# aikiriao/AAD

Measured on AMD Instinct MI355X. Metric: Msamples/s encode+decode, 48 kHz stereo 4-bit, higher is better.
Workload: dtype int32

## Files before the change

### aad_amd/capi.py

```python
import ctypes as C
import os

import numpy as np


class AADApiResult:
    OK = 0
    INVALID_ARGUMENT = 1
    INVALID_FORMAT = 2
    INSUFFICIENT_BUFFER = 3
    INSUFFICIENT_DATA = 4
    PARAMETER_NOT_SET = 5
    NG = 6
    _names = {0: "OK", 1: "INVALID_ARGUMENT", 2: "INVALID_FORMAT", 3: "INSUFFICIENT_BUFFER",
              4: "INSUFFICIENT_DATA", 5: "PARAMETER_NOT_SET", 6: "NG"}

    @classmethod
    def name(cls, v):
        return cls._names.get(int(v), str(v))


class AADHeaderInfo(C.Structure):
    _fields_ = [("format_version", C.c_uint32), ("codec_version", C.c_uint32),
                ("num_channels", C.c_uint16), ("num_samples", C.c_uint32),
                ("sampling_rate", C.c_uint32), ("bits_per_sample", C.c_uint16),
                ("block_size", C.c_uint16), ("num_samples_per_block", C.c_uint32),
                ("ch_process_method", C.c_int)]


class AADEncodeParameter(C.Structure):
    _fields_ = [("num_channels", C.c_uint16), ("sampling_rate", C.c_uint32),
                ("bits_per_sample", C.c_uint16), ("max_block_size", C.c_uint16),
                ("ch_process_method", C.c_int), ("num_encode_trials", C.c_uint8)]


class AADHipStreamDesc(C.Structure):
    _fields_ = [("pcm_offset", C.c_uint64), ("data_offset", C.c_uint64),
                ("data_size", C.c_uint64), ("num_samples", C.c_uint32), ("reserved", C.c_uint32)]


class AADHipSegmentation(C.Structure):
    _fields_ = [("segment_blocks", C.c_uint32), ("warmup_blocks", C.c_uint32)]


class AADHipPlanarLayout(C.Structure):
    _fields_ = [("sample_type", C.c_int32), ("reserved", C.c_uint32), ("channel_stride", C.c_uint64)]


class AADHipPlanarOutput(C.Structure):
    _fields_ = [("sample_type", C.c_int32), ("reserved", C.c_uint32), ("stream_stride", C.c_uint64), ("channel_stride", C.c_uint64)]


class AADHipRowStats(C.Structure):
    _fields_ = [("sum_sq", C.c_uint64), ("sum_abs", C.c_uint64), ("max_abs", C.c_uint64), ("count", C.c_uint64)]


class AADHipLaneState(C.Structure):
    _fields_ = [("weight", C.c_int32 * 4), ("history", C.c_int32 * 4),
                ("stepsize_index", C.c_int32), ("quantize_error", C.c_int32)]


STREAM_DESC_DTYPE = np.dtype([("pcm_offset", "<u8"), ("data_offset", "<u8"), ("data_size", "<u8"),
                              ("num_samples", "<u4"), ("reserved", "<u4")])
ERROR_STATS_DTYPE = np.dtype([("rms_error", "<f8"), ("mean_abs_error", "<f8"), ("max_abs_error", "<f8")])
WINDOW_DTYPE = np.dtype([("stream", "<i8"), ("first_frame", "<i8")])
SAMPLE_INT16, SAMPLE_FLOAT32 = 0, 1
RECONSTRUCT_DECODED, RECONSTRUCT_RESIDUAL = 0, 1
OPTION_LANE_MAPPING, OPTION_TRIAL_LANES, OPTION_STAGING_THREADS, OPTION_TILE_KBYTES, OPTION_COMPARE_ORDER = 0, 1, 2, 3, 4
LANE_MAPPINGS = {"auto": 0, "dense": 1, "quad": 2, "quad-fused": 3, "dense-tiled": 4}
TRIAL_LANES = {"dual": 0, "single": 1}
OPTION_SIMD_ROLE = 5
SIMD_ROLE_OFF = -1
LANE_STATE_DTYPE = np.dtype([("weight", "<i4", (4,)), ("history", "<i4", (4,)),
                             ("stepsize_index", "<i4"), ("quantize_error", "<i4")])

_PKG_DIR = os.path.dirname(os.path.abspath(__file__))
LIBRARY_PATH = os.environ.get("AAD_HIP_LIBRARY", os.path.join(_PKG_DIR, "libaad_hip.so"))

LEGACY_SYMBOLS = [
    "AADEncoder_CalculateBlockSize", "AADEncoder_EncodeHeader", "AADEncoder_CalculateWorkSize",
    "AADEncoder_Create", "AADEncoder_Destroy", "AADEncoder_SetEncodeParameter", "AADEncoder_EncodeWhole",
    "AADDecoder_DecodeHeader", "AADDecoder_CalculateWorkSize", "AADDecoder_Create", "AADDecoder_Destroy",
    "AADDecoder_SetHeader", "AADDecoder_DecodeBlock", "AADDecoder_DecodeWhole",
]
HIP_SYMBOLS = [
    "AADHip_GetDeviceCount", "AADHip_ContextCreate", "AADHip_ContextDestroy", "AADHip_ContextSynchronize",
    "AADHip_ContextLastError", "AADHip_ContextSignalNextRun", "AADHip_SignalNextRunSupported", "AADHip_ContextSetOption", "AADHip_CalculateEncodedSize", "AADHip_EncodePlanCreate",
    "AADHip_EncodePlanDestroy", "AADHip_EncodePlanRun", "AADHip_DecodePlanCreate", "AADHip_DecodePlanDestroy",
    "AADHip_DecodePlanRun", "AADHip_EncodeBatch", "AADHip_DecodeBatch",
    "AADHip_ReconstructPlanCreate", "AADHip_ReconstructPlanDestroy", "AADHip_ReconstructPlanRun",
    "AADHip_ReconstructBatch", "AADHip_SegmentedEncodePlanCreate", "AADHip_SegmentedEncodeBatch",
    "AADHip_SegmentedReconstructPlanCreate", "AADHip_SegmentedReconstructBatch",
    "AADHip_WindowDecodePlanCreate", "AADHip_WindowDecodePlanDestroy", "AADHip_WindowDecodePlanRun",
    "AADHip_WindowDecodePlanRunStats", "AADHip_MixedWindowDecodePlanCreate", "AADHip_ChannelMixWindowDecodePlanCreate",
    "AADHip_PlanarEncodePlanCreate", "AADHip_PlanarEncodePlanRun",
    "AADHip_PlanarReconstructPlanCreate", "AADHip_PlanarReconstructPlanRun", "AADHip_PlanarReconstructPlanRunStats",
    "AADHip_WindowReconstructPlanCreate", "AADHip_WindowReconstructPlanDestroy", "AADHip_WindowReconstructPlanRun",
]
WAV_SYMBOLS = ["AADWav_ParseHeader", "AADWav_WriteHeader", "AADWav_ConvertToPcm16"]
SYNTH_SYMBOLS = ["AADSynth_Generate"]


class AADWavInfo(C.Structure):
    _fields_ = [("format_tag", C.c_uint16), ("num_channels", C.c_uint16), ("sampling_rate", C.c_uint32),
                ("bits_per_sample", C.c_uint16), ("num_samples", C.c_uint32), ("data_offset", C.c_uint64),
                ("data_size", C.c_uint64)]


def _declare_legacy(lib):
    u8p, i32pp = C.POINTER(C.c_uint8), C.POINTER(C.POINTER(C.c_int32))
    lib.AADEncoder_CalculateBlockSize.argtypes = [C.c_uint16, C.c_uint16, C.c_uint32,
                                                  C.POINTER(C.c_uint16), C.POINTER(C.c_uint32)]
    lib.AADEncoder_CalculateBlockSize.restype = C.c_int
    lib.AADEncoder_EncodeHeader.argtypes = [C.POINTER(AADHeaderInfo), u8p, C.c_uint32]
    lib.AADEncoder_EncodeHeader.restype = C.c_int
    lib.AADEncoder_CalculateWorkSize.argtypes = [C.c_uint16]
    lib.AADEncoder_CalculateWorkSize.restype = C.c_int32
    lib.AADEncoder_Create.argtypes = [C.c_uint16, C.c_void_p, C.c_int32]
    lib.AADEncoder_Create.restype = C.c_void_p
    lib.AADEncoder_Destroy.argtypes = [C.c_void_p]
    lib.AADEncoder_Destroy.restype = None
    lib.AADEncoder_SetEncodeParameter.argtypes = [C.c_void_p, C.POINTER(AADEncodeParameter)]
    lib.AADEncoder_SetEncodeParameter.restype = C.c_int
    lib.AADEncoder_EncodeWhole.argtypes = [C.c_void_p, i32pp, C.c_uint32, u8p, C.c_uint32, C.POINTER(C.c_uint32)]
    lib.AADEncoder_EncodeWhole.restype = C.c_int
    lib.AADDecoder_DecodeHeader.argtypes = [u8p, C.c_uint32, C.POINTER(AADHeaderInfo)]
    lib.AADDecoder_DecodeHeader.restype = C.c_int
    lib.AADDecoder_CalculateWorkSize.argtypes = []
    lib.AADDecoder_CalculateWorkSize.restype = C.c_int32
    lib.AADDecoder_Create.argtypes = [C.c_void_p, C.c_int32]
    lib.AADDecoder_Create.restype = C.c_void_p
    lib.AADDecoder_Destroy.argtypes = [C.c_void_p]
    lib.AADDecoder_Destroy.restype = None
    lib.AADDecoder_SetHeader.argtypes = [C.c_void_p, C.POINTER(AADHeaderInfo)]
    lib.AADDecoder_SetHeader.restype = C.c_int
    lib.AADDecoder_DecodeBlock.argtypes = [C.c_void_p, u8p, C.c_uint32, i32pp, C.c_uint32, C.c_uint32,
                                           C.POINTER(C.c_uint32)]
    lib.AADDecoder_DecodeBlock.restype = C.c_int
    lib.AADDecoder_DecodeWhole.argtypes = [C.c_void_p, u8p, C.c_uint32, i32pp, C.c_uint32, C.c_uint32]
    lib.AADDecoder_DecodeWhole.restype = C.c_int


def _declare_hip(lib):
    vp = C.c_void_p
    lib.AADHip_GetDeviceCount.argtypes = []
    lib.AADHip_GetDeviceCount.restype = C.c_int32
    lib.AADHip_ContextCreate.argtypes = [C.c_int32, vp, C.POINTER(vp)]
    lib.AADHip_ContextCreate.restype = C.c_int
    lib.AADHip_ContextDestroy.argtypes = [vp]
    lib.AADHip_ContextDestroy.restype = None
    lib.AADHip_ContextSynchronize.argtypes = [vp]
    lib.AADHip_ContextSynchronize.restype = C.c_int
    lib.AADHip_ContextLastError.argtypes = [vp]
    lib.AADHip_ContextLastError.restype = C.c_char_p
    lib.AADHip_ContextSignalNextRun.argtypes = [vp, vp, vp]
    lib.AADHip_ContextSignalNextRun.restype = C.c_int
    lib.AADHip_SignalNextRunSupported.argtypes = []
    lib.AADHip_SignalNextRunSupported.restype = C.c_int32
    lib.AADHip_ContextSetOption.argtypes = [vp, C.c_int32, C.c_int32]
    lib.AADHip_ContextSetOption.restype = C.c_int
    lib.AADHip_CalculateEncodedSize.argtypes = [C.POINTER(AADEncodeParameter), C.c_uint32]
    lib.AADHip_CalculateEncodedSize.restype = C.c_uint64
    lib.AADHip_EncodePlanCreate.argtypes = [vp, C.POINTER(AADEncodeParameter), C.c_uint32, vp, C.POINTER(vp)]
    lib.AADHip_EncodePlanCreate.restype = C.c_int
    lib.AADHip_SegmentedEncodePlanCreate.argtypes = [vp, C.POINTER(AADEncodeParameter), C.POINTER(AADHipSegmentation), C.c_uint32, vp,
                                                     C.POINTER(vp)]
    lib.AADHip_SegmentedEncodePlanCreate.restype = C.c_int
    lib.AADHip_PlanarEncodePlanCreate.argtypes = [vp, C.POINTER(AADEncodeParameter), C.POINTER(AADHipPlanarLayout),
                                                  C.POINTER(AADHipSegmentation), C.c_uint32, vp, C.POINTER(vp)]
    lib.AADHip_PlanarEncodePlanCreate.restype = C.c_int
    lib.AADHip_PlanarEncodePlanRun.argtypes = [vp, vp, vp, vp]
    lib.AADHip_PlanarEncodePlanRun.restype = C.c_int
    lib.AADHip_PlanarReconstructPlanCreate.argtypes = [vp, C.POINTER(AADEncodeParameter), C.POINTER(AADHipPlanarLayout),
                                                       C.POINTER(AADHipPlanarOutput), C.POINTER(AADHipSegmentation), C.c_uint32, vp,
                                                       C.POINTER(vp)]
    lib.AADHip_PlanarReconstructPlanCreate.restype = C.c_int
    lib.AADHip_PlanarReconstructPlanRun.argtypes = [vp, vp, vp, vp, vp]
    lib.AADHip_PlanarReconstructPlanRun.restype = C.c_int
    lib.AADHip_PlanarReconstructPlanRunStats.argtypes = [vp, vp, vp, vp, vp, vp]
    lib.AADHip_PlanarReconstructPlanRunStats.restype = C.c_int
    lib.AADHip_WindowReconstructPlanCreate.argtypes = [vp, C.POINTER(AADEncodeParameter), C.POINTER(AADHipPlanarLayout),
                                                       C.POINTER(AADHipSegmentation), C.c_uint32, vp, C.POINTER(vp)]
    lib.AADHip_WindowReconstructPlanCreate.restype = C.c_int
    lib.AADHip_WindowReconstructPlanDestroy.argtypes = [vp]
    lib.AADHip_WindowReconstructPlanDestroy.restype = None
    lib.AADHip_WindowReconstructPlanRun.argtypes = [vp, vp, C.c_uint64, vp, C.c_uint32, C.c_uint64, vp, C.POINTER(AADHipPlanarOutput),
                                                    vp, vp]
    lib.AADHip_WindowReconstructPlanRun.restype = C.c_int
    lib.AADHip_EncodePlanDestroy.argtypes = [vp]
    lib.AADHip_EncodePlanDestroy.restype = None
    lib.AADHip_EncodePlanRun.argtypes = [vp, vp, vp, vp]
    lib.AADHip_EncodePlanRun.restype = C.c_int
    lib.AADHip_DecodePlanCreate.argtypes = [vp, C.POINTER(AADHeaderInfo), C.c_int32, C.c_uint32, vp, C.POINTER(vp)]
    lib.AADHip_DecodePlanCreate.restype = C.c_int
    lib.AADHip_DecodePlanDestroy.argtypes = [vp]
    lib.AADHip_DecodePlanDestroy.restype = None
    lib.AADHip_DecodePlanRun.argtypes = [vp, vp, vp]
    lib.AADHip_DecodePlanRun.restype = C.c_int
    lib.AADHip_WindowDecodePlanCreate.argtypes = [vp, C.POINTER(AADHeaderInfo), C.c_int32, C.c_uint32, vp, C.POINTER(vp)]
    lib.AADHip_WindowDecodePlanCreate.restype = C.c_int
    lib.AADHip_MixedWindowDecodePlanCreate.argtypes = [vp, C.c_uint32, C.c_int32, C.c_uint32, vp, vp, C.POINTER(vp)]
    lib.AADHip_MixedWindowDecodePlanCreate.restype = C.c_int
    lib.AADHip_ChannelMixWindowDecodePlanCreate.argtypes = [vp, C.c_uint32, C.c_int32, C.c_uint32, vp, vp, C.POINTER(vp)]
    lib.AADHip_ChannelMixWindowDecodePlanCreate.restype = C.c_int
    lib.AADHip_WindowDecodePlanDestroy.argtypes = [vp]
    lib.AADHip_WindowDecodePlanDestroy.restype = None
    lib.AADHip_WindowDecodePlanRun.argtypes = [vp, vp, C.c_uint64, vp, C.c_uint32, C.c_int32, vp]
    lib.AADHip_WindowDecodePlanRun.restype = C.c_int
    lib.AADHip_WindowDecodePlanRunStats.argtypes = [vp, vp, C.c_uint64, vp, C.c_uint32, C.c_int32, vp, vp]
    lib.AADHip_WindowDecodePlanRunStats.restype = C.c_int
    lib.AADHip_EncodeBatch.argtypes = [vp, C.POINTER(AADEncodeParameter), C.c_uint32, vp, vp, vp, vp, vp, vp]
    lib.AADHip_EncodeBatch.restype = C.c_int
    lib.AADHip_DecodeBatch.argtypes = [vp, C.c_uint32, vp, vp, vp, vp, vp]
    lib.AADHip_DecodeBatch.restype = C.c_int
    lib.AADHip_ReconstructPlanCreate.argtypes = [vp, C.POINTER(AADEncodeParameter), C.c_uint32, vp, C.POINTER(vp)]
    lib.AADHip_ReconstructPlanCreate.restype = C.c_int
    lib.AADHip_ReconstructPlanDestroy.argtypes = [vp]
    lib.AADHip_ReconstructPlanDestroy.restype = None
    lib.AADHip_ReconstructPlanRun.argtypes = [vp, vp, vp, vp, C.c_int32, vp]
    lib.AADHip_ReconstructPlanRun.restype = C.c_int
    lib.AADHip_ReconstructBatch.argtypes = [vp, C.POINTER(AADEncodeParameter), C.c_uint32, vp, vp, C.c_int32, vp, vp]
    lib.AADHip_ReconstructBatch.restype = C.c_int
    lib.AADHip_SegmentedEncodeBatch.argtypes = [vp, C.POINTER(AADEncodeParameter), C.POINTER(AADHipSegmentation), C.c_uint32, vp, vp,
                                                vp, vp, vp]
    lib.AADHip_SegmentedEncodeBatch.restype = C.c_int
    lib.AADHip_SegmentedReconstructPlanCreate.argtypes = [vp, C.POINTER(AADEncodeParameter), C.POINTER(AADHipSegmentation), C.c_uint32,
                                                          vp, C.POINTER(vp)]
    lib.AADHip_SegmentedReconstructPlanCreate.restype = C.c_int
    lib.AADHip_SegmentedReconstructBatch.argtypes = [vp, C.POINTER(AADEncodeParameter), C.POINTER(AADHipSegmentation), C.c_uint32, vp,
                                                     vp, C.c_int32, vp, vp]
    lib.AADHip_SegmentedReconstructBatch.restype = C.c_int
    lib.AADWav_ParseHeader.argtypes = [vp, C.c_uint64, C.POINTER(AADWavInfo)]
    lib.AADWav_ParseHeader.restype = C.c_int
    lib.AADWav_WriteHeader.argtypes = [vp, C.c_uint32, C.c_uint16, C.c_uint32, C.c_uint32]
    lib.AADWav_WriteHeader.restype = C.c_int
    lib.AADWav_ConvertToPcm16.argtypes = [vp, C.c_uint16, C.c_uint64, vp]
    lib.AADWav_ConvertToPcm16.restype = C.c_int


def load_library(path=None, hip=True):
    path = path or LIBRARY_PATH
    if not os.path.exists(path):
        raise FileNotFoundError(
            "%s is missing - the HIP extension has not been built (run __graft_entry__.build())" % path)
    if hip:
        try:
            import torch
        except ImportError:
            pass
    lib = C.CDLL(path)
    _declare_legacy(lib)
# ... 101 lines not shown
```

### aad_amd/csrc/aad_hip_engine.hip

```cpp
#include <hip/hip_runtime.h>

#include <cstdio>
#include <cstdlib>
#include <cstring>
#include <algorithm>
#include <condition_variable>
#include <functional>
#include <mutex>
#include <new>
#include <thread>
#include <vector>

#include "../../include/aad_hip.h"
#include "aad_compare.hip.h"
#include "aad_launch.h"
#include "aad_decode.hip.h"
#include "aad_decode_window.hip.h"
#include "aad_decode_window_mixed.hip.h"
#include "aad_decode_window_channel_mix.hip.h"
#include "aad_encode.hip.h"
#include "aad_encode_launch.hip.h"
#include "aad_format.h"
#include "aad_hip_internal.h"
#include "aad_tiles.h"
#include "aad_window_reconstruct.hip.h"

namespace aad {
thread_local LaunchSignal tl_launch_signal = {nullptr, nullptr};
}

static_assert(sizeof(AADHipStreamDesc) == sizeof(aad::StreamDesc), "stream table layout");
static_assert(sizeof(AADHipLaneState) == sizeof(aad::LaneStateRecord), "lane state layout");
static_assert(sizeof(AADHipErrorStats) == sizeof(aad::ErrorStatsRecord), "error stats layout");

struct Staging {
  void *host = nullptr, *dev = nullptr;
  size_t cap = 0;
};

struct StagingPool {
  std::vector<std::thread> threads;
  std::mutex lock;
  std::condition_variable work, done;
  std::function<void(unsigned)> job;
  unsigned generation = 0, pending = 0;
  bool stop = false;
};

struct AADHipContext {
  int device;
  hipStream_t stream;
  bool owns_stream;
  char last_error[256];
  Staging in[2], out[2];
  hipEvent_t chunk_done[2];
  hipEvent_t piece_done[3];
  hipStream_t up_stream, down_stream;
  hipEvent_t uploaded[2], computed[2];
  bool have_events, have_pipeline;
  void *d_rc_in, *d_rc_out;
  size_t rc_in_capacity, rc_out_capacity;
  void *d_scratch;
  size_t scratch_capacity;
  int32_t *d_residual;
  uint64_t residual_capacity;
  uint8_t *d_trial;
  uint64_t trial_capacity;
  uint8_t *d_window_images;
  uint64_t window_images_capacity;
  aad::LaunchSignal signal_next;
  bool signal_refused;
  aad::Device device_info;
  aad::Knobs knobs;
  int32_t compare_sequential;
  int64_t tile_bytes;
  void *d_state;
// ... 2188 lines not shown
  if (num_streams == 0) return AAD_APIRESULT_OK;
  for (uint32_t i = 0; i < num_streams; i++)
    if (pcm[i] == nullptr || (out_pcm != nullptr && out_pcm[i] == nullptr)) return AAD_APIRESULT_INVALID_ARGUMENT;
  AADHeaderInfo h;
  std::vector<uint64_t> sizes, footprint(num_streams);
  const AADApiResult checked = host_encode_check(parameter, num_streams, num_samples, nullptr, &h, &sizes);
  if (checked != AAD_APIRESULT_OK) return checked;
  for (uint32_t i = 0; i < num_streams; i++) footprint[i] = reconstruct_footprint(num_samples[i], h.num_channels, sizes[i]);
  if (segmentation != nullptr) {
    std::vector<AADHipStreamDesc> streams(num_streams);
    for (uint32_t i = 0; i < num_streams; i++) streams[i] = AADHipStreamDesc{0, 0, 0, num_samples[i], 0};
    if (aad::segment_chain_count(streams.data(), num_streams, h.num_samples_per_block, segmentation->segment_blocks) > UINT32_MAX) {
      snprintf(ctx->last_error, sizeof(ctx->last_error), "segmented reconstruction: more than %u chains", (unsigned)UINT32_MAX);
      return AAD_APIRESULT_INVALID_ARGUMENT;
    }
  }
  const uint64_t chunk = staging_chunk(ctx);
  uint64_t budget;
  if (!wave_budget(ctx, &budget)) return AAD_APIRESULT_NG;
  AADApiResult rc = AAD_APIRESULT_OK;
  for (uint32_t first = 0; first < num_streams && rc == AAD_APIRESULT_OK;) {
    uint32_t n = 0;
    uint64_t sum = 0;
    while (first + n < num_streams && (n == 0 || sum + footprint[first + n] <= budget)) sum += footprint[first + n++];
    rc = reconstruct_wave(ctx, parameter, segmentation, n, pcm + first, num_samples + first, output_kind, out_pcm ? out_pcm + first : nullptr,
                          stats ? stats + first : nullptr, chunk);
    first += n;
  }
  return rc;
}

}

AADApiResult AADHip_ReconstructBatch(struct AADHipContext *ctx, const struct AADEncodeParameter *parameter,
                                     uint32_t num_streams, const int16_t *const *pcm, const uint32_t *num_samples,
                                     int32_t output_kind, int16_t *const *out_pcm, struct AADHipErrorStats *stats)
{
  if (ctx == nullptr || parameter == nullptr || (num_streams != 0 && (pcm == nullptr || num_samples == nullptr)))
    return AAD_APIRESULT_INVALID_ARGUMENT;
  return reconstruct_batch(ctx, parameter, nullptr, num_streams, pcm, num_samples, output_kind, out_pcm, stats);
}

AADApiResult AADHip_SegmentedReconstructBatch(struct AADHipContext *ctx, const struct AADEncodeParameter *parameter,
                                              const struct AADHipSegmentation *segmentation, uint32_t num_streams,
                                              const int16_t *const *pcm, const uint32_t *num_samples, int32_t output_kind,
                                              int16_t *const *out_pcm, struct AADHipErrorStats *stats)
{
  if (ctx == nullptr || parameter == nullptr || segmentation == nullptr || segmentation->segment_blocks == 0 ||
      (num_streams != 0 && (pcm == nullptr || num_samples == nullptr)))
    return AAD_APIRESULT_INVALID_ARGUMENT;
  return reconstruct_batch(ctx, parameter, segmentation, num_streams, pcm, num_samples, output_kind, out_pcm, stats);
}

#if AAD_PHASE_TIMING
uint32_t AADHipDebug_ReadPhaseTimes(uint64_t *out, uint32_t capacity)
{
  uint32_t n = 0, zero = 0;
  uint64_t host[512];
  (void)hipDeviceSynchronize();
  (void)hipMemcpyFromSymbol(&n, HIP_SYMBOL(aad::g_phase_count), sizeof(n));
  (void)hipMemcpyFromSymbol(host, HIP_SYMBOL(aad::g_phase_times), sizeof(host));
  (void)hipMemcpyToSymbol(HIP_SYMBOL(aad::g_phase_count), &zero, sizeof(zero));
  if (n > capacity) n = capacity;
  memcpy(out, host, sizeof(uint64_t) * n);
  return n;
}
#endif

}
```

### aad_amd/csrc/aad_launch_policy.h

```cpp
#ifndef AAD_LAUNCH_POLICY_H
#define AAD_LAUNCH_POLICY_H

#include <stdint.h>

#include "../../include/aad_hip.h"
#include "aad_lds_layout.h"

namespace aad {

struct Device {
  uint32_t cus, lds_per_cu;
};

struct Knobs {
  int32_t lane_mapping = AAD_HIP_LANE_MAPPING_AUTO;
  int32_t trial_lanes = AAD_HIP_TRIAL_LANES_DUAL;
  int32_t encode_ring = 1;
  int32_t encode_lds_pad = -1;
  int32_t decode_lds_pad = -1;
  uint64_t decode_nt_min = 0;
  int32_t simd_role = AAD_HIP_SIMD_ROLE_OFF;
};

struct EncodeBatch {
// ... 368 lines not shown
  uint32_t channels, bits, mid_side, min_samples_per_block, streams;
};
constexpr uint32_t kMaxChannelMixVariants = 9;
struct ChannelMixVariants {
  uint32_t count;
  ChannelMixVariant v[kMaxChannelMixVariants];
};

inline ChannelMixVariants channel_mix_variants(const ChannelStreamFormat *formats, uint64_t n)
{
  ChannelMixVariant slot[kMaxChannelMixVariants] = {};
  for (uint64_t i = 0; i < n; i++) {
    const ChannelStreamFormat &f = formats[i];
    if (f.bits < 2 || f.bits > 4 || f.source >= kSourceNone) continue;
    const bool mono = f.source == kSourceMono, ms = f.source == kSourceMidSide;
    ChannelMixVariant &s = slot[mono ? 6u + (4u - f.bits) : (4u - f.bits) * 2u + (ms ? 1u : 0u)];
    if (s.streams == 0 || f.samples_per_block < s.min_samples_per_block) s.min_samples_per_block = f.samples_per_block;
    s.channels = mono ? 1u : 2u;
    s.bits = f.bits;
    s.mid_side = ms ? 1u : 0u;
    s.streams++;
  }
  ChannelMixVariants out = {};
  for (const ChannelMixVariant &s : slot)
    if (s.streams != 0) out.v[out.count++] = s;
  return out;
}

struct ChannelMixWindowLaunch {
  bool ok;
  uint32_t count;
  ChannelMixVariant variant[kMaxChannelMixVariants];
  WindowLaunch launch[kMaxChannelMixVariants];
};

inline ChannelMixWindowLaunch plan_channel_mix_window_decode(const Device &d, const Knobs &k, const ChannelMixVariants &variants,
                                                             uint64_t windows, uint32_t frames, uint32_t out_channels)
{
  ChannelMixWindowLaunch m = {};
  ChannelMixVariants vs = variants;
  if (vs.count == 0) vs.v[vs.count++] = ChannelMixVariant{1, 4, 0, frames, 0};
  if (vs.count > kMaxChannelMixVariants || out_channels < 1 || out_channels > 2) return m;
  for (uint32_t i = 0; i < vs.count; i++) {
    m.variant[i] = vs.v[i];
    m.launch[i] = plan_window_decode_into(d, k, WindowBatch{windows, frames, vs.v[i].channels, vs.v[i].bits, vs.v[i].min_samples_per_block},
                                          out_channels);
    if (!m.launch[i].ok) return m;
  }
  m.count = vs.count;
  m.ok = true;
  return m;
}

}

#endif
```

### aad_amd/engine.py

```python
import ctypes as C

import numpy as np

from .capi import (AADApiResult, AADHeaderInfo, AADHipPlanarLayout, AADHipPlanarOutput, AADHipSegmentation, ApiError, ERROR_STATS_DTYPE, LANE_MAPPINGS, LANE_STATE_DTYPE,
                   OPTION_COMPARE_ORDER, OPTION_LANE_MAPPING, OPTION_SIMD_ROLE, OPTION_STAGING_THREADS, OPTION_TILE_KBYTES, OPTION_TRIAL_LANES, RECONSTRUCT_DECODED, RECONSTRUCT_RESIDUAL,
                   SAMPLE_FLOAT32, SAMPLE_INT16, SIMD_ROLE_OFF, STREAM_DESC_DTYPE, TRIAL_LANES, WINDOW_DTYPE, load_library, make_parameter)


def _check(where, rc):
    if rc != AADApiResult.OK:
        raise ApiError(where, rc)


def _round_up(v, a):
    return (v + a - 1) // a * a


class Engine:

    def __init__(self, device=0, stream="torch", lib=None):
        import torch
        if not torch.cuda.is_available():
            raise RuntimeError("aad_amd.Engine needs a HIP device (torch.cuda.is_available() is False)")
        self.torch = torch
        self.lib = lib or load_library()
        self.device = int(device)
        torch.cuda.set_device(self.device)
        if stream == "torch":
            cur = torch.cuda.current_stream(self.device)
            self.stream = cur if cur.cuda_stream != 0 else torch.cuda.Stream(self.device)
        elif stream is None:
            self.stream = torch.cuda.Stream(self.device)
        else:
            self.stream = stream
        self._ctx = C.c_void_p()
        _check("AADHip_ContextCreate",
               self.lib.AADHip_ContextCreate(self.device, self.stream.cuda_stream, C.byref(self._ctx)))

    def _enter(self):
        cur = self.torch.cuda.current_stream(self.device)
        if cur.cuda_stream != self.stream.cuda_stream:
            self.stream.wait_stream(cur)
        return cur

    def _exit(self, cur):
        if cur.cuda_stream != self.stream.cuda_stream:
            cur.wait_stream(self.stream)

    def close(self):
        if self._ctx:
            self.lib.AADHip_ContextDestroy(self._ctx)
            self._ctx = C.c_void_p()

    def __del__(self):
        try:
            self.close()
        except Exception:
            pass

# ... 799 lines not shown
        if self.handle:
            self.runtime().hipEventDestroy(self.handle)
            self.handle = C.c_void_p()

    def __del__(self):
        try:
            self.close()
        except Exception:
            pass


PIPELINE_SIMD_ROLES = True


class SimdRoleAllocator:
    SLOTS = ((0, 1), (2, 3))

    def __init__(self):
        self.taken = [False] * len(self.SLOTS)
        self.holders = [None] * len(self.SLOTS)

    def in_force(self):
        return all(self.taken)

    def acquire(self, apply=None):
        for i, t in enumerate(self.taken):
            if not t:
                self.taken[i] = True
                self.holders[i] = apply
                self._apply_all()
                return i
        return None

    def release(self, slot):
        if slot is not None and self.taken[slot]:
            apply = self.holders[slot]
            self.taken[slot], self.holders[slot] = False, None
            if apply is not None:
                apply(None, None)
            self._apply_all()

    def roles(self, slot):
        return self.SLOTS[slot] if slot is not None and self.taken[slot] and self.in_force() else (None, None)

    def _apply_all(self):
        for i, apply in enumerate(self.holders):
            if self.taken[i] and apply is not None:
                apply(*self.roles(i))


_simd_roles = {}


class EncodeDecodePipeline:

    def __init__(self, enc_engine, dec_engine, param, streams, samples, ring=8, simd_roles=PIPELINE_SIMD_ROLES):
        assert ring >= 2 and ring % 2 == 0
        assert enc_engine.stream.cuda_stream != dec_engine.stream.cuda_stream, "the two contexts need streams of their own"
        torch = enc_engine.torch
        self.torch, self.ring, self.k = torch, ring, 0
        self.enc_engine, self.dec_engine = enc_engine, dec_engine
        self._take_simd_roles(_simd_roles.setdefault(enc_engine.device, SimdRoleAllocator()) if simd_roles else None)
        self.enc = enc_engine.uniform_encode_plan(param, streams, samples)
        self.images = [torch.zeros((streams, self.enc.stride), dtype=torch.uint8, device="cuda:%d" % enc_engine.device)
                       for _ in range(ring)]
        zero = torch.zeros((streams, samples, param.num_channels), dtype=torch.int16, device=self.images[0].device)
        self.enc.run(zero, self.images[0])
        torch.cuda.synchronize()
        self.header = parse_header(bytes(self.images[0][0, :31].cpu().numpy()))
        self.dec = dec_engine.uniform_decode_plan(self.header, streams, self.enc.stride, self.enc.image_size)
        self.encoded = [HipEvent() for _ in range(ring)]
        self.decoded = [torch.cuda.Event() for _ in range(ring)]

    def step(self, pcm, out, timing=None):
        k, ring = self.k, self.ring
        self.k += 1
        b = k % ring
        s_enc, s_dec = self.enc_engine.stream, self.dec_engine.stream
        if k >= ring and k % (ring // 2) == 0:
            s_enc.wait_event(self.decoded[(k - ring // 2 - 1) % ring])
        encoded = self.encoded[b] if timing is None else timing[1]
        self.enc_engine.signal_next(encoded, start=None if timing is None else timing[0])
        self.enc.run(pcm, self.images[b], None, ordered=False)
        encoded.wait_on(s_dec)
        if timing is not None:
            self.dec_engine.signal_next(timing[3], start=timing[2])
        self.dec.run(self.images[b], out, ordered=False)
        self.decoded[b].record(s_dec)
        return self.images[b]

    def close(self):
        self.torch.cuda.synchronize()
        self.enc.close()
        self.dec.close()
        for e in self.encoded:
            e.close()
        self._release_simd_roles()

    def _take_simd_roles(self, allocator):
        self._roles = allocator
        self._role_slot = allocator.acquire(self._set_simd_roles) if allocator is not None else None

    def _set_simd_roles(self, enc_simd, dec_simd):
        self.enc_engine.set_simd_role(enc_simd)
        self.dec_engine.set_simd_role(dec_simd)

    def _release_simd_roles(self):
        if getattr(self, "_role_slot", None) is not None:
            self._roles.release(self._role_slot)
            self._role_slot = None


def parse_header(data):
    if len(data) < 31 or data[:4] != b"AAD\x00":
        raise ApiError("parse_header", AADApiResult.INVALID_FORMAT)
    be = lambda o, n: int.from_bytes(data[o:o + n], "big")
    return AADHeaderInfo(format_version=be(4, 4), codec_version=be(8, 4), num_channels=be(12, 2),
                         num_samples=be(14, 4), sampling_rate=be(18, 4), bits_per_sample=be(22, 2),
                         block_size=be(24, 2), num_samples_per_block=be(26, 4), ch_process_method=data[30])


__all__ = ["Engine", "EncodePlan", "PlanarEncodePlan", "PlanarReconstructPlan", "DecodePlan", "WindowDecodePlan", "EncodeDecodePipeline", "SimdRoleAllocator", "parse_header", "make_parameter", "LANE_STATE_DTYPE", "rmse", "snr_db", "level_dbfs", "select_least_bits"]
```

### include/aad_hip.h

```cpp
#ifndef AAD_HIP_H_INCLUDED
#define AAD_HIP_H_INCLUDED

#include <stdint.h>
#include "aad.h"
#include "aad_encoder.h"

#define AAD_HIP_MAX_NUM_CHANNELS 8

struct AADHipContext;
struct AADHipEncodePlan;
struct AADHipDecodePlan;

struct AADHipStreamDesc {
  uint64_t pcm_offset;
  uint64_t data_offset;
  uint64_t data_size;
  uint32_t num_samples;
  uint32_t reserved;
};

struct AADHipLaneState {
  int32_t weight[4];
  int32_t history[4];
  int32_t stepsize_index;
// ... 22 lines not shown
  AAD_HIP_OPTION_COMPARE_ORDER = 4,
  AAD_HIP_OPTION_SIMD_ROLE = 5
};
enum AADHipSimdRole {
  AAD_HIP_SIMD_ROLE_OFF = -1,
  AAD_HIP_SIMD_ROLE_0 = 0, AAD_HIP_SIMD_ROLE_1 = 1, AAD_HIP_SIMD_ROLE_2 = 2, AAD_HIP_SIMD_ROLE_3 = 3
};
enum AADHipLaneMapping {
  AAD_HIP_LANE_MAPPING_AUTO = 0,
  AAD_HIP_LANE_MAPPING_DENSE = 1,
  AAD_HIP_LANE_MAPPING_QUAD = 2,
  AAD_HIP_LANE_MAPPING_QUAD_FUSED = 3,
  AAD_HIP_LANE_MAPPING_DENSE_TILED = 4
};
enum AADHipTrialLanes {
  AAD_HIP_TRIAL_LANES_DUAL = 0,
  AAD_HIP_TRIAL_LANES_SINGLE = 1
};
AADApiResult AADHip_ContextSetOption(struct AADHipContext *context, int32_t option, int32_t value);

uint64_t AADHip_CalculateEncodedSize(const struct AADEncodeParameter *parameter, uint32_t num_samples);


AADApiResult AADHip_EncodePlanCreate(
    struct AADHipContext *context, const struct AADEncodeParameter *parameter,
    uint32_t num_streams, const struct AADHipStreamDesc *streams,
    struct AADHipEncodePlan **plan);
void AADHip_EncodePlanDestroy(struct AADHipEncodePlan *plan);

AADApiResult AADHip_EncodePlanRun(
    struct AADHipEncodePlan *plan, const int16_t *device_pcm, uint8_t *device_data,
    struct AADHipLaneState *device_state);


struct AADHipSegmentation {
  uint32_t segment_blocks;
  uint32_t warmup_blocks;
};
AADApiResult AADHip_SegmentedEncodePlanCreate(
    struct AADHipContext *context, const struct AADEncodeParameter *parameter,
    const struct AADHipSegmentation *segmentation,
    uint32_t num_streams, const struct AADHipStreamDesc *streams,
    struct AADHipEncodePlan **plan);


AADApiResult AADHip_DecodePlanCreate(
    struct AADHipContext *context, const struct AADHeaderInfo *format, int32_t has_file_header,
    uint32_t num_streams, const struct AADHipStreamDesc *streams,
    struct AADHipDecodePlan **plan);
void AADHip_DecodePlanDestroy(struct AADHipDecodePlan *plan);

AADApiResult AADHip_DecodePlanRun(
    struct AADHipDecodePlan *plan, const uint8_t *device_data, int16_t *device_pcm);


struct AADHipWindow {
  uint64_t stream;
  uint64_t first_frame;
};
enum AADHipSampleType {
  AAD_HIP_SAMPLE_INT16 = 0,
  AAD_HIP_SAMPLE_FLOAT32 = 1
};
struct AADHipWindowDecodePlan;
AADApiResult AADHip_WindowDecodePlanCreate(
    struct AADHipContext *context, const struct AADHeaderInfo *format, int32_t has_file_header,
    uint32_t num_streams, const struct AADHipStreamDesc *streams,
    struct AADHipWindowDecodePlan **plan);
void AADHip_WindowDecodePlanDestroy(struct AADHipWindowDecodePlan *plan);
AADApiResult AADHip_WindowDecodePlanRun(
    struct AADHipWindowDecodePlan *plan, const uint8_t *device_data,
    uint64_t num_windows, const struct AADHipWindow *device_windows,
    uint32_t frames_per_window, int32_t sample_type, void *device_out);

AADApiResult AADHip_MixedWindowDecodePlanCreate(
    struct AADHipContext *context, uint32_t num_channels, int32_t has_file_header,
    uint32_t num_streams, const struct AADHipStreamDesc *streams,
    const struct AADHeaderInfo *formats,
    struct AADHipWindowDecodePlan **plan);

AADApiResult AADHip_ChannelMixWindowDecodePlanCreate(
    struct AADHipContext *context, uint32_t out_channels , int32_t has_file_header,
    uint32_t num_streams, const struct AADHipStreamDesc *streams,
    const struct AADHeaderInfo *formats,
    struct AADHipWindowDecodePlan **plan);

struct AADHipRowStats;
AADApiResult AADHip_WindowDecodePlanRunStats(
    struct AADHipWindowDecodePlan *plan, const uint8_t *device_data,
    uint64_t num_windows, const struct AADHipWindow *device_windows,
    uint32_t frames_per_window, int32_t sample_type,
    void *device_out,
    struct AADHipRowStats *device_stats);


struct AADHipPlanarLayout {
  int32_t sample_type;
  uint32_t reserved;
  uint64_t channel_stride;
};
AADApiResult AADHip_PlanarEncodePlanCreate(
    struct AADHipContext *context, const struct AADEncodeParameter *parameter,
    const struct AADHipPlanarLayout *layout,
    const struct AADHipSegmentation *segmentation,
    uint32_t num_streams, const struct AADHipStreamDesc *streams,
    struct AADHipEncodePlan **plan);
// ... 114 lines not shown
```

Measured before the change: 120,000.

## Move encode/decode step pipeline into native code with alternate-stream ordering

Adds a native StepPipeline that schedules encode and decode across two HIP streams with ring-slot events. Per-step Python stream and event bookkeeping is replaced by one C call. A planner picks an 'alternate' order, which runs encode and decode back-to-back on one stream and alternates streams per step, when both kernels would use no more workgroups than there are CUs. Otherwise it keeps the prior overlap order. This cuts host overhead and cross-stream waits when kernels are too small to fill the GPU, at the cost of extra plans and more complex ordering logic.

```diff
diff --git a/aad_amd/capi.py b/aad_amd/capi.py
--- a/aad_amd/capi.py
+++ b/aad_amd/capi.py
@@ -71,6 +71,7 @@
 TRIAL_LANES = {"dual": 0, "single": 1}
 OPTION_SIMD_ROLE = 5
 SIMD_ROLE_OFF = -1
+STEP_ORDERS = {"auto": -1, "overlap": 0, "alternate": 1}
 LANE_STATE_DTYPE = np.dtype([("weight", "<i4", (4,)), ("history", "<i4", (4,)),
                              ("stepsize_index", "<i4"), ("quantize_error", "<i4")])
 
@@ -96,6 +97,8 @@
     "AADHip_PlanarEncodePlanCreate", "AADHip_PlanarEncodePlanRun",
     "AADHip_PlanarReconstructPlanCreate", "AADHip_PlanarReconstructPlanRun", "AADHip_PlanarReconstructPlanRunStats",
     "AADHip_WindowReconstructPlanCreate", "AADHip_WindowReconstructPlanDestroy", "AADHip_WindowReconstructPlanRun",
+    "AADHip_StepPipelineCreate", "AADHip_StepPipelineRun", "AADHip_StepPipelineDestroy", "AADHip_StepPipelineOrder",
+    "AADHip_StepPipelineImageStride", "AADHip_StepPipelineEncodePlan", "AADHip_StepPipelineDecodePlan",
 ]
 WAV_SYMBOLS = ["AADWav_ParseHeader", "AADWav_WriteHeader", "AADWav_ConvertToPcm16"]
 SYNTH_SYMBOLS = ["AADSynth_Generate"]
@@ -197,6 +200,21 @@
     lib.AADHip_DecodePlanDestroy.restype = None
     lib.AADHip_DecodePlanRun.argtypes = [vp, vp, vp]
     lib.AADHip_DecodePlanRun.restype = C.c_int
+    lib.AADHip_StepPipelineCreate.argtypes = [vp, vp, C.POINTER(AADEncodeParameter), C.c_uint32, C.c_uint32, C.c_uint32, C.POINTER(vp),
+                                              C.c_int32, C.POINTER(vp)]
+    lib.AADHip_StepPipelineCreate.restype = C.c_int
+    lib.AADHip_StepPipelineRun.argtypes = [vp, vp, vp, C.POINTER(vp), C.POINTER(C.c_uint32)]
+    lib.AADHip_StepPipelineRun.restype = C.c_int
+    lib.AADHip_StepPipelineDestroy.argtypes = [vp]
+    lib.AADHip_StepPipelineDestroy.restype = None
+    lib.AADHip_StepPipelineOrder.argtypes = [vp]
+    lib.AADHip_StepPipelineOrder.restype = C.c_int32
+    lib.AADHip_StepPipelineImageStride.argtypes = [vp]
+    lib.AADHip_StepPipelineImageStride.restype = C.c_uint64
+    lib.AADHip_StepPipelineEncodePlan.argtypes = [vp, C.c_uint32]
+    lib.AADHip_StepPipelineEncodePlan.restype = vp
+    lib.AADHip_StepPipelineDecodePlan.argtypes = [vp, C.c_uint32]
+    lib.AADHip_StepPipelineDecodePlan.restype = vp
     lib.AADHip_WindowDecodePlanCreate.argtypes = [vp, C.POINTER(AADHeaderInfo), C.c_int32, C.c_uint32, vp, C.POINTER(vp)]
     lib.AADHip_WindowDecodePlanCreate.restype = C.c_int
     lib.AADHip_MixedWindowDecodePlanCreate.argtypes = [vp, C.c_uint32, C.c_int32, C.c_uint32, vp, vp, C.POINTER(vp)]
diff --git a/aad_amd/csrc/aad_hip_engine.hip b/aad_amd/csrc/aad_hip_engine.hip
--- a/aad_amd/csrc/aad_hip_engine.hip
+++ b/aad_amd/csrc/aad_hip_engine.hip
@@ -22,6 +22,7 @@
 #include "aad_encode_launch.hip.h"
 #include "aad_format.h"
 #include "aad_hip_internal.h"
+#include "aad_step_schedule.h"
 #include "aad_tiles.h"
 #include "aad_window_reconstruct.hip.h"
 
@@ -2316,6 +2317,193 @@
   return reconstruct_batch(ctx, parameter, segmentation, num_streams, pcm, num_samples, output_kind, out_pcm, stats);
 }
 
+
+struct AADHipStepPipeline {
+  AADHipContext *ctx[2];
+  AADHipEncodePlan *enc[2];
+  AADHipDecodePlan *dec[2];
+  aad::StepOrder order;
+  uint32_t ring;
+  uint64_t k, stride, out_elements;
+  std::vector<uint8_t *> images;
+  std::vector<hipEvent_t> own[2];
+  std::vector<hipEvent_t> done[2];
+  const int16_t *last_out;
+};
+
+namespace {
+
+void step_pipeline_free(AADHipStepPipeline *p)
+{
+  for (int q = 0; q < 2; q++) {
+    AADHip_EncodePlanDestroy(p->enc[q]);
+    AADHip_DecodePlanDestroy(p->dec[q]);
+  }
+  for (auto &events : p->own)
+    for (hipEvent_t e : events)
+      if (e != nullptr) (void)hipEventDestroy(e);
+  delete p;
+}
+
+AADApiResult step_pipeline_launch(AADHipStepPipeline *p, aad::StepKernel kernel, uint32_t queue, uint32_t slot, hipEvent_t start,
+                                  hipEvent_t stop, const int16_t *device_pcm, int16_t *device_out)
+{
+  const AADApiResult rc = AADHip_ContextSignalNextRun(p->ctx[queue], start, stop);
+  if (rc != AAD_APIRESULT_OK) return rc;
+  p->done[(int)kernel][slot] = stop;
+  return kernel == aad::StepKernel::Encode ? AADHip_EncodePlanRun(p->enc[queue], device_pcm, p->images[slot], nullptr)
+                                           : AADHip_DecodePlanRun(p->dec[queue], p->images[slot], device_out);
+}
+
+}
+
+AADApiResult AADHip_StepPipelineCreate(struct AADHipContext *ctx0, struct AADHipContext *ctx1, const struct AADEncodeParameter *parameter,
+                                       uint32_t num_streams, uint32_t num_samples, uint32_t ring, uint8_t *const *device_images,
+                                       int32_t order, struct AADHipStepPipeline **pipeline)
+{
+  if (pipeline == nullptr) return AAD_APIRESULT_INVALID_ARGUMENT;
+  *pipeline = nullptr;
+  if (ctx0 == nullptr || ctx1 == nullptr || ctx0 == ctx1 || parameter == nullptr || device_images == nullptr || num_streams == 0 ||
+      !aad::step_ring_ok(ring) || order < AAD_HIP_STEP_ORDER_AUTO || order > AAD_HIP_STEP_ORDER_ALTERNATE)
+    return AAD_APIRESULT_INVALID_ARGUMENT;
+  if (ctx0->device != ctx1->device || ctx0->stream == ctx1->stream) return AAD_APIRESULT_INVALID_ARGUMENT;
+  for (uint32_t i = 0; i < ring; i++)
+    if (device_images[i] == nullptr) return AAD_APIRESULT_INVALID_ARGUMENT;
+  if (ctx0->signal_refused || ctx1->signal_refused) {
+    snprintf(ctx0->last_error, sizeof(ctx0->last_error),
+             "AADHip_StepPipelineCreate: refused, ROC_SYSTEM_SCOPE_SIGNAL=0 (the pipeline orders its two streams with the kernels' own "
+             "completion signals, AADHip_ContextSignalNextRun)");
+    return AAD_APIRESULT_NG;
+  }
+  AADHeaderInfo header;
+  if (AADFormat_ParameterToHeader(parameter, num_samples, AAD_HIP_MAX_NUM_CHANNELS, &header) != AAD_APIRESULT_OK ||
+      !AADFormat_HeaderFieldsValid(&header, AAD_HIP_MAX_NUM_CHANNELS))
+    return AAD_APIRESULT_INVALID_FORMAT;
+  const uint64_t image_size = AADHip_CalculateEncodedSize(parameter, num_samples);
+  if (image_size == 0) return AAD_APIRESULT_INVALID_FORMAT;
+  const uint64_t stride = (image_size + 63u) / 64u * 64u;
+  std::vector<AADHipStreamDesc> table(num_streams);
+  for (uint32_t i = 0; i < num_streams; i++)
+    table[i] = AADHipStreamDesc{(uint64_t)i * num_samples * parameter->num_channels, (uint64_t)i * stride, stride, num_samples, 0};
+
+  AADHipStepPipeline *p = new (std::nothrow) AADHipStepPipeline();
+  if (p == nullptr) return AAD_APIRESULT_NG;
+  p->ctx[0] = ctx0;
+  p->ctx[1] = ctx1;
+  p->ring = ring;
+  p->stride = stride;
+  p->out_elements = (uint64_t)num_streams * num_samples * parameter->num_channels;
+  p->images.assign(device_images, device_images + ring);
+  AADApiResult rc = AADHip_EncodePlanCreate(ctx0, parameter, num_streams, table.data(), &p->enc[0]);
+  for (auto &d : table) d.data_size = image_size;
+  if (rc == AAD_APIRESULT_OK) rc = AADHip_DecodePlanCreate(ctx1, &header, 1, num_streams, table.data(), &p->dec[1]);
+  if (rc == AAD_APIRESULT_OK) {
+    const aad::EncodeArgs &e = p->enc[0]->run.args;
+    const aad::DecodeArgs &d = p->dec[1]->args;
+    p->order = (aad::StepOrder)aad::plan_step_order(
+        ctx0->device_info, ctx0->knobs, aad::EncodeBatch{e.bits, e.channels, e.num_streams, e.trials, e.block_size, e.ring_ok != 0},
+        aad::DecodeBatch{d.total_blocks, d.num_streams, d.channels, d.bits, d.samples_per_block, d.block_size, d.code_phase_uniform,
+                         d.pcm_aligned16 != 0, true, d.stream_stores != 0},
+        order);
+    if (p->order == aad::StepOrder::Alternate) {
+      rc = AADHip_DecodePlanCreate(ctx0, &header, 1, num_streams, table.data(), &p->dec[0]);
+      for (auto &t : table) t.data_size = stride;
+      if (rc == AAD_APIRESULT_OK) rc = AADHip_EncodePlanCreate(ctx1, parameter, num_streams, table.data(), &p->enc[1]);
+    }
+  }
+  if (rc == AAD_APIRESULT_OK) {
+    DeviceGuard guard(ctx0);
+    bool ok = guard.ok;
+    for (int kernel = 0; kernel < 2 && ok; kernel++) {
+      p->own[kernel].assign(ring, nullptr);
+      p->done[kernel].assign(ring, nullptr);
+      for (uint32_t i = 0; i < ring && ok; i++)
+        ok = hip_ok(ctx0, hipEventCreateWithFlags(&p->own[kernel][i], hipEventDisableTiming), "hipEventCreateWithFlags");
+    }
+    if (!ok) rc = AAD_APIRESULT_NG;
+  }
+  if (rc != AAD_APIRESULT_OK) {
+    step_pipeline_free(p);
+    return rc;
+  }
+  *pipeline = p;
+  return AAD_APIRESULT_OK;
+}
+
+AADApiResult AADHip_StepPipelineRun(struct AADHipStepPipeline *p, const int16_t *device_pcm, int16_t *device_out,
+                                    void *const *timing_events, uint32_t *slot)
+{
+  if (p == nullptr || device_pcm == nullptr || device_out == nullptr) return AAD_APIRESULT_INVALID_ARGUMENT;
+  hipEvent_t timing[4] = {nullptr, nullptr, nullptr, nullptr};
+  if (timing_events != nullptr)
+    for (int i = 0; i < 4; i++) {
+      if (timing_events[i] == nullptr) return AAD_APIRESULT_INVALID_ARGUMENT;
+      timing[i] = static_cast<hipEvent_t>(timing_events[i]);
+    }
+  const uint64_t k = p->k;
+  const bool overlaps = p->last_out != nullptr && device_out < p->last_out + p->out_elements && p->last_out < device_out + p->out_elements;
+  const aad::StepSchedule s = aad::step_schedule(k, p->ring, p->order, overlaps);
+  DeviceGuard guard(p->ctx[0]);
+  if (!guard.ok) return AAD_APIRESULT_NG;
+  auto wait_before = [&](aad::StepKernel before) {
+    for (uint32_t i = 0; i < s.num_waits; i++) {
+      const aad::StepWait &w = s.waits[i];
+      if (w.before != before) continue;
+      AADHipContext *ctx = p->ctx[w.queue];
+      const hipEvent_t event = p->done[(int)w.of][w.step % p->ring];
+      if (event == nullptr) {
+        snprintf(ctx->last_error, sizeof(ctx->last_error), "AADHip_StepPipelineRun: step %llu carries no event to wait for",
+                 (unsigned long long)w.step);
+        return false;
+      }
+      if (!hip_ok(ctx, hipStreamWaitEvent(ctx->stream, event, 0), "hipStreamWaitEvent")) return false;
+    }
+    return true;
+  };
+  auto own_event = [&](aad::StepKernel kernel) {
+    return aad::step_kernel_is_waited_for(k, p->ring, p->order, kernel) ? p->own[(int)kernel][s.slot] : (hipEvent_t) nullptr;
+  };
+  if (!wait_before(aad::StepKernel::Encode)) return AAD_APIRESULT_NG;
+  AADApiResult rc = step_pipeline_launch(p, aad::StepKernel::Encode, s.encode_queue, s.slot, timing[0],
+                                         timing_events != nullptr ? timing[1] : own_event(aad::StepKernel::Encode), device_pcm, device_out);
+  if (rc != AAD_APIRESULT_OK) return rc;
+  if (!wait_before(aad::StepKernel::Decode)) return AAD_APIRESULT_NG;
+  rc = step_pipeline_launch(p, aad::StepKernel::Decode, s.decode_queue, s.slot, timing[2],
+                            timing_events != nullptr ? timing[3] : own_event(aad::StepKernel::Decode), device_pcm, device_out);
+  if (rc != AAD_APIRESULT_OK) return rc;
+  if (timing_events != nullptr && p->order == aad::StepOrder::Overlap && own_event(aad::StepKernel::Decode) != nullptr) {
+    AADHipContext *ctx = p->ctx[s.decode_queue];
+    if (!hip_ok(ctx, hipEventRecord(own_event(aad::StepKernel::Decode), ctx->stream), "hipEventRecord")) return AAD_APIRESULT_NG;
+    p->done[(int)aad::StepKernel::Decode][s.slot] = own_event(aad::StepKernel::Decode);
+  }
+  p->last_out = device_out;
+  p->k = k + 1;
+  if (slot != nullptr) *slot = s.slot;
+  return AAD_APIRESULT_OK;
+}
+
+void AADHip_StepPipelineDestroy(struct AADHipStepPipeline *p)
+{
+  if (p == nullptr) return;
+  DeviceGuard guard(p->ctx[0]);
+  if (guard.ok) {
+    (void)hipStreamSynchronize(p->ctx[0]->stream);
+    (void)hipStreamSynchronize(p->ctx[1]->stream);
+  }
+  step_pipeline_free(p);
+}
+
+int32_t AADHip_StepPipelineOrder(const struct AADHipStepPipeline *p) { return p != nullptr ? (int32_t)p->order : AAD_HIP_STEP_ORDER_AUTO; }
+uint64_t AADHip_StepPipelineImageStride(const struct AADHipStepPipeline *p) { return p != nullptr ? p->stride : 0; }
+struct AADHipEncodePlan *AADHip_StepPipelineEncodePlan(const struct AADHipStepPipeline *p, uint32_t queue)
+{
+  return p != nullptr && queue < 2 ? p->enc[queue] : nullptr;
+}
+struct AADHipDecodePlan *AADHip_StepPipelineDecodePlan(const struct AADHipStepPipeline *p, uint32_t queue)
+{
+  return p != nullptr && queue < 2 ? p->dec[queue] : nullptr;
+}
+
 #if AAD_PHASE_TIMING
 uint32_t AADHipDebug_ReadPhaseTimes(uint64_t *out, uint32_t capacity)
 {
diff --git a/aad_amd/csrc/aad_launch_policy.h b/aad_amd/csrc/aad_launch_policy.h
--- a/aad_amd/csrc/aad_launch_policy.h
+++ b/aad_amd/csrc/aad_launch_policy.h
@@ -444,6 +444,16 @@
   return m;
 }
 
+inline int32_t plan_step_order(const Device &d, const Knobs &k, const EncodeBatch &e, const DecodeBatch &b, int32_t option)
+{
+  if (option == AAD_HIP_STEP_ORDER_OVERLAP || option == AAD_HIP_STEP_ORDER_ALTERNATE) return option;
+  const EncodeLaunch pe = plan_encode(d, k, e);
+  const DecodeLaunch pd = plan_decode(d, k, b);
+  const bool starved = (pe.kernel == EncodeKernel::Quad || pe.kernel == EncodeKernel::QuadDual) && pe.grid <= d.cus &&
+                       (pd.kernel == DecodeKernel::SplitLds || pd.kernel == DecodeKernel::SplitScratch) && pd.grid <= d.cus;
+  return starved ? AAD_HIP_STEP_ORDER_ALTERNATE : AAD_HIP_STEP_ORDER_OVERLAP;
+}
+
 }
 
 #endif
diff --git a/aad_amd/csrc/aad_step_schedule.h b/aad_amd/csrc/aad_step_schedule.h
--- /dev/null
+++ b/aad_amd/csrc/aad_step_schedule.h
@@ -0,0 +1,54 @@
+#ifndef AAD_STEP_SCHEDULE_H
+#define AAD_STEP_SCHEDULE_H
+
+#include <stdint.h>
+
+namespace aad {
+
+enum class StepOrder : int32_t { Overlap = 0, Alternate = 1 };
+enum class StepKernel : uint8_t { Encode = 0, Decode = 1 };
+
+struct StepWait {
+  uint32_t queue;
+  StepKernel before;
+  StepKernel of;
+  uint64_t step;
+};
+
+constexpr uint32_t kMaxStepWaits = 2;
+
+struct StepSchedule {
+  uint32_t encode_queue, decode_queue, slot, num_waits;
+  StepWait waits[kMaxStepWaits];
+};
+
+inline bool step_ring_ok(uint32_t ring) { return ring >= 2u && ring % 2u == 0u; }
+
+inline StepSchedule step_schedule(uint64_t k, uint32_t ring, StepOrder order, bool out_overlaps_previous)
+{
+  StepSchedule s{};
+  s.slot = (uint32_t)(k % ring);
+  if (order == StepOrder::Alternate) {
+    s.encode_queue = s.decode_queue = (uint32_t)(k & 1u);
+    if (k > 0 && out_overlaps_previous) s.waits[s.num_waits++] = StepWait{s.decode_queue, StepKernel::Decode, StepKernel::Decode, k - 1};
+    return s;
+  }
+  s.encode_queue = 0;
+  s.decode_queue = 1;
+  const uint32_t half = ring / 2u;
+  if (k >= ring && k % half == 0) s.waits[s.num_waits++] = StepWait{0, StepKernel::Encode, StepKernel::Decode, k - half - 1};
+  s.waits[s.num_waits++] = StepWait{1, StepKernel::Decode, StepKernel::Encode, k};
+  return s;
+}
+
+inline bool step_kernel_is_waited_for(uint64_t k, uint32_t ring, StepOrder order, StepKernel kernel)
+{
+  if (order == StepOrder::Alternate) return kernel == StepKernel::Decode;
+  if (kernel == StepKernel::Encode) return true;
+  const uint32_t half = ring / 2u;
+  return (k + 1) % half == 0;
+}
+
+}
+
+#endif
diff --git a/aad_amd/engine.py b/aad_amd/engine.py
--- a/aad_amd/engine.py
+++ b/aad_amd/engine.py
@@ -1,10 +1,11 @@
 import ctypes as C
+import os
 
 import numpy as np
 
 from .capi import (AADApiResult, AADHeaderInfo, AADHipPlanarLayout, AADHipPlanarOutput, AADHipSegmentation, ApiError, ERROR_STATS_DTYPE, LANE_MAPPINGS, LANE_STATE_DTYPE,
                    OPTION_COMPARE_ORDER, OPTION_LANE_MAPPING, OPTION_SIMD_ROLE, OPTION_STAGING_THREADS, OPTION_TILE_KBYTES, OPTION_TRIAL_LANES, RECONSTRUCT_DECODED, RECONSTRUCT_RESIDUAL,
-                   SAMPLE_FLOAT32, SAMPLE_INT16, SIMD_ROLE_OFF, STREAM_DESC_DTYPE, TRIAL_LANES, WINDOW_DTYPE, load_library, make_parameter)
+                   SAMPLE_FLOAT32, SAMPLE_INT16, SIMD_ROLE_OFF, STEP_ORDERS, STREAM_DESC_DTYPE, TRIAL_LANES, WINDOW_DTYPE, load_library, make_parameter)
 
 
 def _check(where, rc):
@@ -910,49 +911,65 @@
 _simd_roles = {}
 
 
+class _BorrowedEncodePlan(EncodePlan):
+
+    def close(self):
+        self.handle = None
+
+
+class _BorrowedDecodePlan(DecodePlan):
+    def close(self):
+        self.handle = None
+
+
 class EncodeDecodePipeline:
 
-    def __init__(self, enc_engine, dec_engine, param, streams, samples, ring=8, simd_roles=PIPELINE_SIMD_ROLES):
+    def __init__(self, enc_engine, dec_engine, param, streams, samples, ring=8, simd_roles=PIPELINE_SIMD_ROLES, order=None):
         assert ring >= 2 and ring % 2 == 0
         assert enc_engine.stream.cuda_stream != dec_engine.stream.cuda_stream, "the two contexts need streams of their own"
         torch = enc_engine.torch
         self.torch, self.ring, self.k = torch, ring, 0
         self.enc_engine, self.dec_engine = enc_engine, dec_engine
+        self._handle = C.c_void_p()
         self._take_simd_roles(_simd_roles.setdefault(enc_engine.device, SimdRoleAllocator()) if simd_roles else None)
-        self.enc = enc_engine.uniform_encode_plan(param, streams, samples)
-        self.images = [torch.zeros((streams, self.enc.stride), dtype=torch.uint8, device="cuda:%d" % enc_engine.device)
+        size = enc_engine.encoded_size(param, samples)
+        if size == 0:
+            raise ApiError("AADHip_CalculateEncodedSize", AADApiResult.INVALID_FORMAT)
+        stride = _round_up(size, 64)
+        self.images = [torch.zeros((streams, stride), dtype=torch.uint8, device="cuda:%d" % enc_engine.device)
                        for _ in range(ring)]
+        if order is None:
+            order = os.environ.get("AAD_HIP_STEP_ORDER", "auto")
+        lib = enc_engine.lib
+        pointers = (C.c_void_p * ring)(*[t.data_ptr() for t in self.images])
+        _check("AADHip_StepPipelineCreate",
+               lib.AADHip_StepPipelineCreate(enc_engine._ctx, dec_engine._ctx, C.byref(param), streams, samples, ring, pointers,
+                                             STEP_ORDERS[order], C.byref(self._handle)))
+        assert lib.AADHip_StepPipelineImageStride(self._handle) == stride
+        self.order = {v: n for n, v in STEP_ORDERS.items()}[lib.AADHip_StepPipelineOrder(self._handle)]
+        self.enc = _BorrowedEncodePlan(enc_engine, C.c_void_p(lib.AADHip_StepPipelineEncodePlan(self._handle, 0)), param, None)
+        self.enc.image_size, self.enc.stride = size, stride
         zero = torch.zeros((streams, samples, param.num_channels), dtype=torch.int16, device=self.images[0].device)
         self.enc.run(zero, self.images[0])
         torch.cuda.synchronize()
         self.header = parse_header(bytes(self.images[0][0, :31].cpu().numpy()))
-        self.dec = dec_engine.uniform_decode_plan(self.header, streams, self.enc.stride, self.enc.image_size)
-        self.encoded = [HipEvent() for _ in range(ring)]
-        self.decoded = [torch.cuda.Event() for _ in range(ring)]
+        self.dec = _BorrowedDecodePlan(dec_engine, C.c_void_p(lib.AADHip_StepPipelineDecodePlan(self._handle, 1)), self.header, None)
+        self._slot = C.c_uint32()
 
     def step(self, pcm, out, timing=None):
-        k, ring = self.k, self.ring
+        events = None if timing is None else (C.c_void_p * 4)(*[t.handle.value for t in timing])
+        _check("AADHip_StepPipelineRun",
+               self.enc_engine.lib.AADHip_StepPipelineRun(self._handle, pcm.data_ptr(), out.data_ptr(), events, C.byref(self._slot)))
         self.k += 1
-        b = k % ring
-        s_enc, s_dec = self.enc_engine.stream, self.dec_engine.stream
-        if k >= ring and k % (ring // 2) == 0:
-            s_enc.wait_event(self.decoded[(k - ring // 2 - 1) % ring])
-        encoded = self.encoded[b] if timing is None else timing[1]
-        self.enc_engine.signal_next(encoded, start=None if timing is None else timing[0])
-        self.enc.run(pcm, self.images[b], None, ordered=False)
-        encoded.wait_on(s_dec)
-        if timing is not None:
-            self.dec_engine.signal_next(timing[3], start=timing[2])
-        self.dec.run(self.images[b], out, ordered=False)
-        self.decoded[b].record(s_dec)
-        return self.images[b]
+        return self.images[self._slot.value]
 
     def close(self):
         self.torch.cuda.synchronize()
         self.enc.close()
         self.dec.close()
-        for e in self.encoded:
-            e.close()
+        if self._handle:
+            self.enc_engine.lib.AADHip_StepPipelineDestroy(self._handle)
+            self._handle = C.c_void_p()
         self._release_simd_roles()
 
     def _take_simd_roles(self, allocator):
diff --git a/include/aad_hip.h b/include/aad_hip.h
--- a/include/aad_hip.h
+++ b/include/aad_hip.h
@@ -98,6 +98,26 @@
 
 AADApiResult AADHip_DecodePlanRun(
     struct AADHipDecodePlan *plan, const uint8_t *device_data, int16_t *device_pcm);
+
+
+struct AADHipStepPipeline;
+enum AADHipStepOrder {
+  AAD_HIP_STEP_ORDER_AUTO = -1,
+  AAD_HIP_STEP_ORDER_OVERLAP = 0,
+  AAD_HIP_STEP_ORDER_ALTERNATE = 1
+};
+AADApiResult AADHip_StepPipelineCreate(
+    struct AADHipContext *context0, struct AADHipContext *context1, const struct AADEncodeParameter *parameter,
+    uint32_t num_streams, uint32_t num_samples, uint32_t ring, uint8_t *const *device_images, int32_t order,
+    struct AADHipStepPipeline **pipeline);
+AADApiResult AADHip_StepPipelineRun(
+    struct AADHipStepPipeline *pipeline, const int16_t *device_pcm, int16_t *device_out, void *const *timing_events,
+    uint32_t *slot);
+void AADHip_StepPipelineDestroy(struct AADHipStepPipeline *pipeline);
+int32_t AADHip_StepPipelineOrder(const struct AADHipStepPipeline *pipeline);
+uint64_t AADHip_StepPipelineImageStride(const struct AADHipStepPipeline *pipeline);
+struct AADHipEncodePlan *AADHip_StepPipelineEncodePlan(const struct AADHipStepPipeline *pipeline, uint32_t queue);
+struct AADHipDecodePlan *AADHip_StepPipelineDecodePlan(const struct AADHipStepPipeline *pipeline, uint32_t queue);
 
 
 struct AADHipWindow {
```

Result: no change. 120,600, median of 4 (+0.4%).
